# AbbVie-ComputationalGenomics/SAIGEgds

Measured on AMD Instinct MI355X. Metric: variants/sec seqAssocGLMM_SPA at N=430K; achieved HBM GB/s vs roofline, higher is better.
Workload: dtype f64

## Files before the change

### saigegds_amd/csrc/host_init.h

```cpp
extern "C" const char *sgx_version(void) { return "saigehip 0.1 (gfx950)"; }
extern "C" const char *sgx_last_error(void) { return g_err.c_str(); }

extern "C" int sgx_device_count(void)
{
	int n = 0;
	if (hipGetDeviceCount(&n) != hipSuccess) return 0;
	return n;
}

extern "C" size_t sgx_row_stride(int32_t n_samp)
{
	return (size_t)((n_samp + 511) / 512) * 128;
}

static double thr_or(double v, double dflt) { return std::isfinite(v) ? v : dflt; }

extern "C" int sgx_set_thresholds(sgx_handle *h, double maf, double mac, double missing,
	double spa_pval)
{
	if (!h) return fail(SGX_EINVAL, "sgx_set_thresholds: NULL handle");
	h->md.thr_maf = thr_or(maf, -1);
	h->md.thr_mac = thr_or(mac, -1);
	h->md.thr_missing = thr_or(missing, 1);
	h->md.thr_spa = thr_or(spa_pval, 0.05);
// ... 148 lines not shown
		return fail(SGX_EINVAL, "sgx_init: device %d out of range (0..%d)", device, ndev - 1);

	sgx_handle *h = new sgx_handle();
	h->device = device;
	int rc = set_dev(h);
	if (rc) { delete h; return rc; }
	const int P = 2 * K + 2;
	const bool quant = m->trait == SGX_TRAIT_QUANT;
	const int KP = (K + 2) & ~1;
	std::vector<double> F((size_t)N * P), X((size_t)N * K), y(m->y, m->y + N),
		mu(m->mu, m->mu + N), mu2(m->mu2, m->mu2 + N), XM((size_t)N * KP, 0.0);
	long double xmu[KMAX] = {0}, xsum[KMAX] = {0};
	for (int i = 0; i < N; i++) {
		const double w = quant ? 1.0 : m->mu2[i];
		double *f = &F[(size_t)i * P];
		for (int k = 0; k < K; k++) {
			f[k] = m->t_XVX_inv_XV[(size_t)i * K + k];
			f[K + k] = w * m->t_X[(size_t)i * K + k];
			X[(size_t)i * K + k] = m->t_X[(size_t)i * K + k];
			XM[(size_t)i * KP + k] = m->t_X[(size_t)i * K + k];
			xmu[k] += (long double)m->t_X[(size_t)i * K + k] * m->mu[i];
			xsum[k] += (long double)m->t_X[(size_t)i * K + k];
		}
		XM[(size_t)i * KP + K] = m->mu[i];
		f[2 * K] = m->y_mu[i];
		f[2 * K + 1] = w;
	}
	std::vector<int8_t> Fl;
	std::vector<long long> Qt;
	if ((double)N * 4.0 * 384.0 < 2147483647.0) {
		MfEpi &ep = h->mfe;
		const int CS = 2 * K, CW = 2 * K + 1;
		const int ngrp = (N + 15) / 16;
		const int ntile = 2 * ((ngrp + 31) / 32);
		const size_t ngrp_pad = (size_t)ntile * 16;
		ep.derive_c = quant && fit_xvx_inverse(m, ep.XVXi) ? 1 : 0;
		std::vector<int> order = {CS, CW};
		for (int k = 0; k < K; k++) order.push_back(K + k);
		if (!ep.derive_c) for (int k = 0; k < K; k++) order.push_back(k);
		for (int k = 0; k < K; k++) { ep.cgrp[k] = 0; ep.ccol[k] = 0; ep.climb[k] = 0; }
		bool range_ok = true;
		auto limbs_for = [&](int c) -> int {
			if (c == CW && quant) return 1;
			long double sum = 0; double mx = 0;
			for (int i = 0; i < N; i++) { const double a = std::fabs(F[(size_t)i * P + c]); sum += a; mx = std::max(mx, a); }
			const double range = sum > 0 ? mx / (double)(sum / N) : 1.0;
			if (!(range <= 4194304.0)) range_ok = false;
			int nl = c >= 2 * K ? MF_NLIMB : (c >= K ? MF_LIMB_E : MF_LIMB_A);
			if (range > 64.0) nl = std::max(nl, MF_LIMB_E);
			if (range > 16384.0) nl = MF_NLIMB;
			if (N < 16384) nl = std::min(MF_NLIMB, nl + 1);
			return nl;
		};
		int used = 1;
		for (int c : order) {
			const int nl = limbs_for(c);
			ep.cgrp[c] = 0; ep.ccol[c] = (unsigned char)(used - 1); ep.climb[c] = (unsigned char)nl;
			used += nl;
		}
		if (range_ok) {
		const int nbfv = (used + 15) / 16;
		h->mf_nbfv[0] = nbfv;
		ep.ngroups = 1;
		ep.goff[0] = 0;
		ep.gncol[0] = 16 * (nbfv + 1);
		ep.acc_stride = ep.gncol[0];
		ep.col_ones = used - 1;
		ep.col_b1 = 16 * nbfv;
		h->mf[0].ntile = ntile;
		Fl.assign(ngrp_pad * ep.gncol[0] * 16, 0);
		Qt.assign((size_t)N * P, 0);
		auto at = [&](int i, int col) -> int8_t & {
			return Fl[((size_t)(i / 16) * ep.gncol[0] + col) * 16 + s3_pos(i % 16)];
		};
		for (int c = 0; c < P; c++) {
			const int cc = ep.ccol[c], nl = ep.climb[c];
			if (nl == 0) { ep.escale[c] = 0; ep.ftot_hi[c] = ep.ftot_lo[c] = 0; continue; }
			double mx = 0;
			for (int i = 0; i < N; i++) mx = std::max(mx, std::fabs(F[(size_t)i * P + c]));
			int ex = 0;
			if (mx > 0) (void)std::frexp(mx, &ex);
			ep.escale[c] = (quant && c == CW) ? 2 : 8 * nl - 2 - ex;
			__int128 tot = 0;
			for (int i = 0; i < N; i++) {
				const int sc = s3_scale(i % 16);
				const long long d0 = std::llrint(std::ldexp(F[(size_t)i * P + c], ep.escale[c]) / sc);
				const long long q = d0 * sc;
				Qt[(size_t)i * P + c] = q;
				tot += q;
				long long rem = d0;
				for (int l = 0; l < nl; l++) {
					long long d = (l < nl - 1) ? (((rem + 128) & 255) - 128) : rem;
					rem = (rem - d) >> 8;
					at(i, cc + l) = (int8_t)d;
					if (c == CW) at(i, ep.col_b1 + l) = (int8_t)d;
				}
			}
			const __int128 two32 = ((__int128)1) << 32;
			__int128 hi = tot / two32, lo = tot - hi * two32;
			if (lo < 0) { lo += two32; hi -= 1; }
			ep.ftot_hi[c] = (long long)hi; ep.ftot_lo[c] = (long long)lo;
		}
		for (int i = 0; i < N; i++) {
			const int8_t d = (int8_t)(4 / s3_scale(i % 16));
			at(i, ep.col_ones) = d;
			at(i, ep.col_b1 + ep.climb[CW]) = d;
		}
		h->mf_ok = true;
		}
	}
	DevModel &md = h->md;
	md.N = N; md.K = K; md.P = P; md.quant = quant;
	md.tau0 = m->tau[0]; md.r = m->var_ratio;
	sgx_set_thresholds(h, m->maf, m->mac, m->missing, m->spa_pval);
	{
		double l2min = INFINITY;
		for (int i = 0; i < N; i++) {
			const double mi = m->mu[i];
			if (mi > 0 && mi < 1) { const double lg = std::log(mi / (1 - mi)); l2min = std::min(l2min, lg * lg); }
		}
		md.spa_xmax = std::isfinite(l2min) ? 0.25 * std::sqrt(l2min + M_PI * M_PI) : 0.0;
	}
	for (int k = 0; k < K; k++) {
		double mx = 0;
		for (int i = 0; i < N; i++) mx = std::max(mx, std::fabs(m->t_X[(size_t)i * K + k]));
		md.Xabs[k] = mx;
	}
	for (int a = 0; a < K * K; a++) md.XVX[a] = m->XVX[a];
	for (int a = 0; a < K; a++) { md.S_a[a] = m->S_a[a]; md.Xmu[a] = (double)xmu[a]; md.Xsum[a] = (double)xsum[a]; }
#define TRY(x) do { rc = (x); if (rc) { sgx_free(h); return rc; } } while (0)
	TRY(dev_upload(&h->dF, F));
	TRY(dev_upload(&h->dX, X));
	TRY(dev_upload(&h->dy, y));
	TRY(dev_upload(&h->dmu, mu));
	TRY(dev_upload(&h->dmu2, mu2));
	TRY(dev_upload(&h->dXM, XM));
	if (h->mf_ok) {
		std::vector<uint8_t> Flu(Fl.begin(), Fl.end());
		TRY(dev_upload(&h->dFl, Flu));
		h->mf[0].Fl = h->dFl;
		TRY(dev_upload(&h->dQ, Qt));
	}
	md.F = h->dF; md.X = h->dX; md.y = h->dy; md.mu = h->dmu; md.mu2 = h->dmu2; md.XM = h->dXM;
	rc = alloc_workspace(h);
	if (rc) { sgx_free(h); return rc; }
#undef TRY
	*out = h;
	return SGX_OK;
}

extern "C" int sgx_score_layout(sgx_handle *h, int32_t *limbs, int32_t n_limbs, int32_t *n_groups)
{
	if (!h || !n_groups) return fail(SGX_EINVAL, "sgx_score_layout: NULL argument");
	*n_groups = h->mf_ok ? h->mfe.ngroups : 0;
	for (int c = 0; limbs && c < n_limbs; c++) limbs[c] = (h->mf_ok && c < h->md.P) ? h->mfe.climb[c] : 0;
	return SGX_OK;
}

extern "C" void sgx_free(sgx_handle *h)
// ... 69 lines not shown
```

### saigegds_amd/csrc/kern_score3.h

```cpp
#pragma once
#include <type_traits>

#ifndef S3_V4I_DEFINED
#define S3_V4I_DEFINED
typedef int s3_v4i __attribute__((ext_vector_type(4)));
#endif

#include "s3_layout.h"

template <int OFF> __device__ __forceinline__ void s3_ds_read(s3_v4i &dst, uint32_t addr)
{
	asm volatile("ds_read_b128 %0, %1 offset:%2" : "=v"(dst) : "v"(addr), "n"(OFF));
}
template <int N> __device__ __forceinline__ void s3_lgkm_wait(s3_v4i &reg) { asm volatile("s_waitcnt lgkmcnt(%1)" : "+v"(reg) : "n"(N)); }
__device__ __forceinline__ void s3_tie(s3_v4i &reg) { asm volatile("" : "+v"(reg)); }
#define S3_DS_READ(dst, addr, off) s3_ds_read<(off)>(dst, addr)
#define S3_LGKM_WAIT(n, reg) s3_lgkm_wait<(n)>(reg)
#define S3_TIE(reg) s3_tie(reg)

template <int I, int N, typename F>
__device__ __forceinline__ void s3_static_for(F &&f)
{
	if constexpr (I < N) { f(std::integral_constant<int, I>()); s3_static_for<I + 1, N>(f); }
}

#ifndef S3_AUX_ROWS
#define S3_AUX_ROWS 2
#endif
#define S3_WAITCNT_VM(n) __builtin_amdgcn_s_waitcnt(((n) & 0xF) | (((n) >> 4) << 14) | (0x7 << 4) | (0xF << 8))

template <int OP>
__device__ __forceinline__ void s3_unpack_op(uint32_t w, uint32_t &w4, s3_v4i &val, s3_v4i &b1)
{
	if constexpr (OP == 0) w4 = w >> 4;
	else if constexpr (OP == 1) val[0] = (int)(w & 0x03030303u);
	else if constexpr (OP == 2) val[1] = (int)(w & 0x0C0C0C0Cu);
	else if constexpr (OP == 3) val[2] = (int)(w4 & 0x03030303u);
	else if constexpr (OP == 4) val[3] = (int)(w4 & 0x0C0C0C0Cu);
	else if constexpr (OP == 5) b1[0] = (int)(w & 0x02020202u);
	else if constexpr (OP == 6) b1[1] = (int)(w & 0x08080808u);
	else if constexpr (OP == 7) b1[2] = (int)(w4 & 0x02020202u);
	else if constexpr (OP == 8) b1[3] = (int)(w4 & 0x08080808u);
}
#define S3_UNPACK3_OPS 15
template <int OP>
__device__ __forceinline__ void s3_unpack3_op(uint32_t w, uint32_t &w4, uint32_t &t, uint32_t &t4, s3_v4i &val, s3_v4i &b1, s3_v4i &mis)
{
	if constexpr (OP < 9) s3_unpack_op<OP>(w, w4, val, b1);
	else if constexpr (OP == 9) t = w >> 1;
	else if constexpr (OP == 10) t4 = w4 >> 1;
	else if constexpr (OP == 11) mis[0] = (int)(w & t & 0x01010101u);
	else if constexpr (OP == 12) mis[1] = (int)(w & t & 0x04040404u);
	else if constexpr (OP == 13) mis[2] = (int)(w4 & t4 & 0x01010101u);
	else if constexpr (OP == 14) mis[3] = (int)(w4 & t4 & 0x04040404u);
}

template <int NAF>
struct s3_one {
	static constexpr int NM = 7 * NAF, NOPT = S3_UNPACK3_OPS * NAF, DL = 2, NK = 3 * NOPT;
	static constexpr int piece_of(int m) { return m < NAF ? m : m < 3 * NAF ? (m - NAF) / 2 : (m - 3 * NAF) / 4; }
	static constexpr int frag_of(int m) { return m < NAF ? 3 : m < 3 * NAF ? 0 : 1 + ((m - 3 * NAF) & 3) / 2; }
	static constexpr int plane_of(int m) { return m < NAF ? 2 : m < 3 * NAF ? (m - NAF) & 1 : (m - 3 * NAF) & 1; }
	static constexpr int chunk_of(int m) { return m < 3 * NAF ? 0 : 1; }
	static constexpr int slot_of(int m) { return m < NAF ? 0 : m < 3 * NAF ? 1 : ((m - 3 * NAF) & 3) / 2; }
	static constexpr int frag(int ch, int j) { return ch == 0 ? (j == 0 ? 3 : 0) : 1 + j; }
	static constexpr bool enters(int m) { return m == 0 || m == 3 * NAF; }
	static constexpr int piece(int i) { return i < 7 * NAF ? i / 7 : (i - 7 * NAF) / 8; }
	static constexpr int op(int i)
	{
		const int head[7] = {0, 9, 10, 5, 6, 7, 8}, tail[8] = {1, 2, 3, 4, 11, 12, 13, 14};
		return i < 7 * NAF ? head[i % 7] : tail[(i - 7 * NAF) % 8];
	}
	static constexpr int earliest(int d, int i)
	{
		const int base = NM * (d - 1);
		if (i < 7 * NAF) return base + (i % 7 >= 3 ? i / 7 : 0);
		const int q = i - 7 * NAF;
		return base + 3 * NAF + 4 * (q / 8) + (q % 8 < 4 ? 2 : 3);
	}
	static constexpr int deadline(int d, int i)
	{
		const int base = NM * d;
		if (i < 7 * NAF) return i % 7 >= 3 ? base + i / 7 : 1 << 30;
		const int q = i - 7 * NAF;
		return base + NAF + 2 * (q / 8) + (q % 8 < 4 ? 0 : 1);
	}
	static constexpr int slot(int k)
	{
		int s = 0;
		for (int j = 0; j <= k; j++) {
			const int d = 1 + j / NOPT, i = j % NOPT, t = NM * (d - 1) + i * NM / NOPT + DL, e = earliest(d, i);
			s = s > t ? s : t;
			s = s > e ? s : e;
		}
		return s;
	}
	static constexpr int first(int g) { int k = 0; while (k < NK && slot(k) < g) k++; return k; }
	static constexpr bool ok()
	{
		for (int k = 0; k < NK; k++)
			if (slot(k) >= deadline(1 + k / NOPT, k % NOPT) || slot(k) >= 4 * NM) return false;
		return true;
	}
};

template <int NBF, int NAF, int NC, int NLA, int NLB, int DA, int DB, int ABL = 0, int NCB = 1, int NBUF_ = 2, int RM = 0, bool MISS = false>
__global__ void __launch_bounds__(64 * (NC + NLA + NLB), (NC + NLA + NLB + 3) / 4)
score3_kernel(const uint8_t *__restrict__ A, const uint8_t *__restrict__ Fl, S3Plan pl, int *__restrict__ out, unsigned long long *__restrict__ stamps)
{
#if __HIP_DEVICE_COMPILE__
	static_assert(NC % NCB == 0 && NCB >= 1 && NCB <= 4, "consumer waves = variant groups x column groups");
	constexpr int NCV = NC / NCB;
	constexpr int NBWMAX = (NBF + NCB - 1) / NCB;
	constexpr int NCOL = 16 * NBF;
	constexpr int TILE_BYTES = 16 * NCOL * 16;
	constexpr int NPB = TILE_BYTES / 1024;
	constexpr int NPA = NCV * NAF;
	constexpr int RA = DA + 1, RB = DB + 1;
	constexpr int SLOT_A = (RM == 1 ? 2 : 1) * NPA * 1024;
	static_assert(DA >= 1 && DB >= 1, "at least one tile ahead");
	extern __shared__ __attribute__((aligned(16))) uint8_t s3_smem[];

	const int tid = threadIdx.x, lane = tid & 63, wid = tid >> 6;
	const int x = blockIdx.x & 7, y = blockIdx.x >> 3;
	const int g = x % pl.ng, i = y * (8 / pl.ng) + x / pl.ng;
	const int nk = pl.rf + (i < pl.rem * pl.f ? 1 : 0);
	const int T0 = 2 * (int)((long long)g * (pl.ntile / 2) / pl.ng), T1 = 2 * (int)((long long)(g + 1) * (pl.ntile / 2) / pl.ng);
	unsigned long long st0 = 0, sr0 = 0;
	if (ABL & 16) { st0 = __builtin_amdgcn_s_memtime(); sr0 = __builtin_amdgcn_s_memrealtime(); }

	struct Pos { int k, t, t1, vtile, id; };
	auto pos_set = [&](Pos &p, int k) {
		p.k = k;
		if (k >= nk) return;
		if (k < pl.rf) { p.vtile = k * pl.wpg + i; p.t = T0; p.t1 = T1; p.id = g * pl.ipg + p.vtile; }
		else {
			const int q = i % pl.f, vv = i / pl.f, len = T1 - T0;
			p.vtile = pl.rf * pl.wpg + vv;
			p.t = T0 + 2 * (q * (len / 2) / pl.f); p.t1 = T0 + 2 * ((q + 1) * (len / 2) / pl.f);
			p.id = g * pl.ipg + pl.rf * pl.wpg + i;
		}
	};
	auto pos_next = [&](Pos &p) { if (++p.t >= p.t1) pos_set(p, p.k + 1); };
	Pos pc;
	pos_set(pc, 0);

	if (wid >= NC) {
		const bool rows = wid < NC + NLA;
		const int l = __builtin_amdgcn_readfirstlane(rows ? wid - NC : wid - NC - NLA);
		const int voff = (rows ? s3_dma_lane(lane) : lane) * 16;
		const unsigned rm_bpv = (unsigned)pl.bpv;
		Pos pa = pc;
		int sl = 0;
		int ahead = 0;
		if (rows && RM == 1) {
			constexpr int PLO = NPA / NLA, NHI = NPA % NLA;
			static_assert(2 * (PLO + 1) * (DA > 1 ? DA - 1 : 1) < 64, "vmcnt range");
			const int li = lane >> 3, lj = lane & 7;
			const int rlast = pl.nrow - 1 - 16 * (pl.nfrag - 1);
			unsigned vo[2], vol[2];
#pragma unroll
			for (int h = 0; h < 2; h++) {
				const unsigned c = (unsigned)(lj ^ ((li >> 1) | (h << 2)));
				vo[h] = (unsigned)(8 * h + li) * rm_bpv + c * 16u;
				vol[h] = (unsigned)min(8 * h + li, rlast) * rm_bpv + c * 16u;
			}
			auto issue = [&]() {
// ... 54 lines not shown
#pragma unroll
			for (int d = 0; d < DA; d++) if (pa.k < nk) { issue(); ahead++; }
			while (pc.k < nk) {
				if (ahead == DA && DA > 1) { if (l < NHI) S3_WAITCNT_VM((PLO + 1) * (DA - 1)); else S3_WAITCNT_VM(PLO * (DA - 1)); }
				else S3_WAITCNT_VM(0);
				__builtin_amdgcn_s_barrier();
				ahead--;
				if (pa.k < nk) { issue(); ahead++; }
				pos_next(pc);
			}
		} else {
			constexpr int PLO = NPB / NLB, NHI = NPB % NLB;
			static_assert((PLO + 1) * (DB - 1) < 64, "vmcnt range");
			const __amdgpu_buffer_rsrc_t rsB = __builtin_amdgcn_make_buffer_rsrc((void *)Fl, 0, 0xFFFFFFFFu, 0x00020000);
			auto issue = [&]() {
#pragma unroll
				for (int j = 0; j <= PLO; j++) {
					const int b = l + j * NLB;
					if (b >= NPB || (ABL & 4)) break;
					__builtin_amdgcn_raw_ptr_buffer_load_lds(rsB, (__attribute__((address_space(3))) void *)(s3_smem + sl * TILE_BYTES + b * 1024),
						16, voff, pa.t * TILE_BYTES + b * 1024, 0, 0);
				}
				sl = sl + 1 == RB ? 0 : sl + 1;
				pos_next(pa);
			};
#pragma unroll
			for (int d = 0; d < DB; d++) if (pa.k < nk) { issue(); ahead++; }
			while (pc.k < nk) {
				if (ahead == DB && DB > 1) { if (l < NHI) S3_WAITCNT_VM((PLO + 1) * (DB - 1)); else S3_WAITCNT_VM(PLO * (DB - 1)); }
				else S3_WAITCNT_VM(0);
				__builtin_amdgcn_s_barrier();
				ahead--;
				if (pa.k < nk) { issue(); ahead++; }
				pos_next(pc);
			}
		}
		return;
	}

	const int r = lane & 15, kg = lane >> 4;
	const int vg = __builtin_amdgcn_readfirstlane(wid / NCB), cgr = __builtin_amdgcn_readfirstlane(wid % NCB);
	const uint32_t smem_lds = (uint32_t)(uintptr_t)(__attribute__((address_space(3))) uint8_t *)s3_smem;
	const uint32_t ring_lds = smem_lds + RB * TILE_BYTES + vg * (NAF * 1024) + lane * 16;
	const int rm_sig = ((r & 7) >> 1) | ((r >> 3) << 2);
	const uint32_t ring_rm = smem_lds + RB * TILE_BYTES + vg * (NAF * 2048) + (uint32_t)(r >> 3) * 1024u + (uint32_t)(r & 7) * 128u;
	const uint32_t ring_rm0 = ring_rm + (uint32_t)(kg ^ rm_sig) * 16u, ring_rm1 = ring_rm + (uint32_t)((4 + kg) ^ rm_sig) * 16u;

	auto consume = [&](auto CG) {
		constexpr int cg = decltype(CG)::value;
		constexpr int B0 = cg * NBWMAX;
		constexpr int NBW = (NBF - B0 < NBWMAX) ? NBF - B0 : NBWMAX;
		constexpr bool HASB1 = B0 + NBW == NBF;
		static_assert(NBW >= 1, "empty column group");
		const uint32_t bt_lds = smem_lds + (4 * kg * NCOL + r) * 16 + B0 * 256;

		s3_v4i acc[NAF][NBW];
#pragma unroll
		for (int f = 0; f < NAF; f++)
#pragma unroll
			for (int b = 0; b < NBW; b++) acc[f][b] = (s3_v4i){0, 0, 0, 0};

		constexpr int BCH = NBUF_ > 2 ? 1 : NCB > 1 ? (NBW <= 2 ? NBW : 2) : (NBF <= 4 ? NBF : (NBF >= 9 ? 2 : (NBF % 3 == 0 ? 3 : 4)));
		constexpr int NBUF = NBUF_;
		constexpr bool PIPE = NCB == 1 && NBF <= 8;
		constexpr int NCH = (NBW + BCH - 1) / BCH;
		constexpr int NM = NAF * NBW;
		constexpr int NV = HASB1 ? 4 * NAF : 0, NW = 5 * NAF;
		constexpr int BLV = HASB1 ? NBW - 2 : NBW - 1;
		constexpr int MB = HASB1 ? ((!PIPE && NBW >= 3) ? (NBW - 2) * NAF : (NBW - 1) * NAF) : 0;
		static_assert(!HASB1 || NBW >= 2 || NCB == 1, "a column group of the b1 fragment alone has no slot for its unpack");

		int sa = 0, sb = 0;
		int par = 0;
		while (pc.k < nk) {
			__builtin_amdgcn_sched_barrier(0);
			__builtin_amdgcn_s_barrier();
			__builtin_amdgcn_sched_barrier(0);
			const uint32_t a_addr = (RM == 1 ? (par ? ring_rm1 : ring_rm0) : ring_lds) + (uint32_t)(sa * SLOT_A);
			constexpr int AFS = RM == 1 ? 2048 : 1024;
			const uint32_t b_addr = bt_lds + (uint32_t)(sb * TILE_BYTES);
			s3_v4i aw[NAF];
			s3_static_for<0, NAF>([&](auto F) { constexpr int f = decltype(F)::value; S3_DS_READ(aw[f], a_addr, f * AFS); });
			s3_v4i bf[NBUF][BCH];
			auto read_chunk = [&](auto CI) {
				constexpr int ci = decltype(CI)::value, u = ci / NCH, b0 = (ci % NCH) * BCH;
				s3_static_for<0, BCH>([&](auto J) {
					constexpr int j = decltype(J)::value;
					if constexpr (b0 + j < NBW) {
						if (ABL & 8) bf[ci % NBUF][j] = (s3_v4i){u, j, r, sa};
						else S3_DS_READ(bf[ci % NBUF][j], b_addr, u * NCOL * 16 + (b0 + j) * 256);
					}
				});
			};
			constexpr int nread_last = NBW - (NCH - 1) * BCH;
			auto nreads = [](int c0, int c1) constexpr { int n = 0; for (int c = c0; c < c1 && c < 4 * NCH; c++) n += (c % NCH == NCH - 1) ? nread_last : BCH; return n; };
			s3_static_for<0, NBUF - 1>([&](auto C) { if constexpr (decltype(C)::value < 4 * NCH) read_chunk(C); });
			if (!(ABL & 8)) { S3_LGKM_WAIT(nreads(0, NBUF - 1), aw[0]); } else { S3_LGKM_WAIT(0, aw[0]); }
#pragma unroll
			for (int f = 1; f < NAF; f++) S3_TIE(aw[f]);
			s3_v4i val[PIPE ? 2 : 1][NAF], b1[NAF];
			uint32_t w4[PIPE ? 2 : 1][NAF];
			if (!(ABL & 1)) {
				s3_static_for<0, (PIPE ? NW : 5)>([&](auto O) {
					constexpr int o = decltype(O)::value, f = o / 5, op = o % 5;
					s3_unpack_op<op>((uint32_t)aw[f][0], w4[0][f], val[0][f], b1[f]);
				});
			}
			__builtin_amdgcn_sched_barrier(0);
			constexpr bool FM = !PIPE && BCH == 2 && nread_last == 2;
			constexpr int M0 = (NCH - 1) * BCH * NAF;
			s3_static_for<0, 4>([&](auto U) {
				constexpr int u = decltype(U)::value;
				constexpr int vb = PIPE ? (u & 1) : 0, vn = PIPE ? ((u + 1) & 1) : 0;
				s3_static_for<0, NM>([&](auto MI) {
					constexpr int m = decltype(MI)::value;
					constexpr bool fm = FM && m >= M0;
					constexpr int b = fm ? (NCH - 1) * BCH + (m - M0) % 2 : m / NAF, f = fm ? (m - M0) / 2 : m % NAF;
					constexpr int ch = b / BCH, ci = u * NCH + ch, j = b % BCH;
					if constexpr (m == ch * BCH * NAF) {
						if constexpr (ci + NBUF - 1 < 4 * NCH) read_chunk(std::integral_constant<int, ci + NBUF - 1>());
						constexpr int inflight = (ABL & 8) ? 0 : nreads(ci + 1, ci + NBUF);
						constexpr int nb = (ch == NCH - 1) ? nread_last : BCH;
						S3_LGKM_WAIT(inflight, bf[ci % NBUF][0]);
#pragma unroll
						for (int jj = 1; jj < nb; jj++) S3_TIE(bf[ci % NBUF][jj]);
					}
					if (ABL & 1) { if (f == 0) acc[0][b][1] ^= bf[ci % NBUF][j][0] ^ aw[b % NAF][u]; }
					else if (HASB1 && b == NBW - 1) acc[f][b] = __builtin_amdgcn_mfma_i32_16x16x64_i8(b1[f], bf[ci % NBUF][j], acc[f][b], 0, 0, 0);
					else acc[f][b] = __builtin_amdgcn_mfma_i32_16x16x64_i8(val[vb][f], bf[ci % NBUF][j], acc[f][b], 0, 0, 0);
					if (!(ABL & 1)) {
						if constexpr (!PIPE && u == 0 && b == 0 && f + 1 < NAF) {
							s3_static_for<0, 5>([&](auto O) {
								constexpr int op = decltype(O)::value;
								s3_unpack_op<op>((uint32_t)aw[f + 1][0], w4[0][f + 1], val[0][f + 1], b1[f + 1]);
							});
						}
						if constexpr (m < MB) {
							s3_static_for<m * NV / MB, (m + 1) * NV / MB>([&](auto O) {
								constexpr int o = decltype(O)::value, ff = o / 4, op = 5 + o % 4;
								s3_unpack_op<op>((uint32_t)aw[ff][u], w4[vb][ff], val[vb][ff], b1[ff]);
							});
						}
						if constexpr (PIPE && u < 3) {
							s3_static_for<m * NW / NM, (m + 1) * NW / NM>([&](auto O) {
								constexpr int o = decltype(O)::value, ff = o / 5, op = o % 5;
								s3_unpack_op<op>((uint32_t)aw[ff][u + 1], w4[vn][ff], val[vn][ff], b1[ff]);
							});
						}
						if constexpr (!PIPE && u < 3) {
							constexpr int lo = !fm ? ((b == BLV || (BLV < 0 && b == 0)) ? 0 : 5) : (HASB1 ? (j == 0 ? 0 : 2) : (j == 1 ? 0 : 5));
							constexpr int hi = !fm ? 5 : (HASB1 && j == 0 ? 2 : 5);
							s3_static_for<lo, hi>([&](auto O) {
								constexpr int op = decltype(O)::value;
								s3_unpack_op<op>((uint32_t)aw[f][u + 1], w4[0][f], val[0][f], b1[f]);
							});
						}
					}
					__builtin_amdgcn_sched_barrier(0);
				});
			});
			if (pc.t + 1 == pc.t1) {
				int *dst = out + ((size_t)pc.id * NC + wid) * (NAF * NBWMAX * 256) + lane;
#pragma unroll
				for (int f = 0; f < NAF; f++)
#pragma unroll
					for (int b = 0; b < NBW; b++)
#pragma unroll
						for (int reg = 0; reg < 4; reg++) {
							dst[((f * NBWMAX + b) * 4 + reg) * 64] = acc[f][b][reg];
							acc[f][b][reg] = 0;
						}
			}
			pos_next(pc);
			if (RM != 1 || par) sa = sa + 1 == RA ? 0 : sa + 1;
			sb = sb + 1 == RB ? 0 : sb + 1;
			par ^= 1;
		}
	};
	auto consume3 = [&]() {
		static_assert(!MISS || NCB == 1, "the three-plane form has one column group");
		constexpr int NBUF = NBUF_;
		constexpr int NBV = NBF - 1;
		constexpr int NVF = 2 * NBV + 1;
		constexpr int NM = NAF * NVF;
		constexpr int NOPT = S3_UNPACK3_OPS * NAF;
		constexpr bool ONE = NBF == 4 && NAF >= 3;
		using S1 = s3_one<NAF>;
		static_assert(!ONE || S1::ok(), "an unpack operation of the one-set schedule lands behind the MFMA that needs it");
		constexpr int BCH = ONE ? 2 : NBF <= 4 ? NBF : 2, NCH = (NBF + BCH - 1) / BCH;
		constexpr int NPS = ONE ? 1 : 2;
		const uint32_t bt_lds = smem_lds + (4 * kg * NCOL + r) * 16;
		s3_v4i acc[NAF][NBF], accm[NAF][NBV > 0 ? NBV : 1];
#pragma unroll
		for (int f = 0; f < NAF; f++) {
#pragma unroll
			for (int b = 0; b < NBF; b++) acc[f][b] = (s3_v4i){0, 0, 0, 0};
#pragma unroll
			for (int b = 0; b < NBV; b++) accm[f][b] = (s3_v4i){0, 0, 0, 0};
		}
		int sa = 0, sb = 0, par = 0;
		while (pc.k < nk) {
			__builtin_amdgcn_sched_barrier(0);
			__builtin_amdgcn_s_barrier();
			__builtin_amdgcn_sched_barrier(0);
			const uint32_t a_addr = (RM == 1 ? (par ? ring_rm1 : ring_rm0) : ring_lds) + (uint32_t)(sa * SLOT_A);
			constexpr int AFS = RM == 1 ? 2048 : 1024;
			const uint32_t b_addr = bt_lds + (uint32_t)(sb * TILE_BYTES);
			s3_v4i aw[NAF];
			s3_static_for<0, NAF>([&](auto F) { constexpr int f = decltype(F)::value; S3_DS_READ(aw[f], a_addr, f * AFS); });
			s3_v4i bf[NBUF][BCH];
			auto read_chunk = [&](auto CI) {
				constexpr int ci = decltype(CI)::value, u = ci / NCH, b0 = (ci % NCH) * BCH;
				s3_static_for<0, BCH>([&](auto J) {
					constexpr int j = decltype(J)::value;
					constexpr int b = ONE ? S1::frag(ci % NCH, j) : b0 + j;
					if constexpr (b0 + j < NBF) S3_DS_READ(bf[ci % NBUF][j], b_addr, u * NCOL * 16 + b * 256);
				});
			};
			constexpr int nread_last = NBF - (NCH - 1) * BCH;
			auto nreads = [](int c0, int c1) constexpr { int n = 0; for (int c = c0; c < c1 && c < 4 * NCH; c++) n += (c % NCH == NCH - 1) ? nread_last : BCH; return n; };
			s3_static_for<0, NBUF - 1>([&](auto C) { if constexpr (decltype(C)::value < 4 * NCH) read_chunk(C); });
			S3_LGKM_WAIT(nreads(0, NBUF - 1), aw[0]);
#pragma unroll
			for (int f = 1; f < NAF; f++) S3_TIE(aw[f]);
			s3_v4i val[NPS][NAF], b1[NPS][NAF], mis[NPS][NAF];
			uint32_t w4[NAF], tt[NAF], m4[NAF];
			s3_static_for<0, NOPT>([&](auto O) {
				constexpr int o = decltype(O)::value, f = o / S3_UNPACK3_OPS, op = o % S3_UNPACK3_OPS;
				s3_unpack3_op<op>((uint32_t)aw[f][0], w4[f], tt[f], m4[f], val[0][f], b1[0][f], mis[0][f]);
			});
			__builtin_amdgcn_sched_barrier(0);
			s3_static_for<0, 4>([&](auto U) {
				constexpr int u = decltype(U)::value, vb = ONE ? 0 : u & 1, vn = ONE ? 0 : (u + 1) & 1;
				s3_static_for<0, NM>([&](auto MI) {
					constexpr int m = decltype(MI)::value, vf = m / NAF;
					constexpr int f = ONE ? S1::piece_of(m) : m % NAF;
					constexpr int b = ONE ? S1::frag_of(m) : vf < 2 * NBV ? vf / 2 : NBV;
					constexpr int plane = ONE ? S1::plane_of(m) : vf < 2 * NBV ? (vf & 1) : 2;
					constexpr int ch = ONE ? S1::chunk_of(m) : b / BCH, ci = u * NCH + ch, j = ONE ? S1::slot_of(m) : b % BCH;
					if constexpr (ONE ? S1::enters(m) : f == 0 && plane != 1 && b % BCH == 0) {
						if constexpr (ci + NBUF - 1 < 4 * NCH) read_chunk(std::integral_constant<int, ci + NBUF - 1>());
						constexpr int inflight = nreads(ci + 1, ci + NBUF);
						constexpr int nb = (ch == NCH - 1) ? nread_last : BCH;
						S3_LGKM_WAIT(inflight, bf[ci % NBUF][0]);
#pragma unroll
						for (int jj = 1; jj < nb; jj++) S3_TIE(bf[ci % NBUF][jj]);
					}
					if constexpr (plane == 0) acc[f][b] = __builtin_amdgcn_mfma_i32_16x16x64_i8(val[vb][f], bf[ci % NBUF][j], acc[f][b], 0, 0, 0);
					else if constexpr (plane == 1) accm[f][b] = __builtin_amdgcn_mfma_i32_16x16x64_i8(mis[vb][f], bf[ci % NBUF][j], accm[f][b], 0, 0, 0);
					else acc[f][b] = __builtin_amdgcn_mfma_i32_16x16x64_i8(b1[vb][f], bf[ci % NBUF][j], acc[f][b], 0, 0, 0);
					if constexpr (ONE) {
						constexpr int g = u * NM + m;
						s3_static_for<S1::first(g), S1::first(g + 1)>([&](auto K) {
							constexpr int k = decltype(K)::value, d = 1 + k / NOPT, i = k % NOPT, ff = S1::piece(i), op = S1::op(i);
							s3_unpack3_op<op>((uint32_t)aw[ff][d], w4[ff], tt[ff], m4[ff], val[0][ff], b1[0][ff], mis[0][ff]);
						});
					} else if constexpr (u < 3) {
						s3_static_for<m * NOPT / NM, (m + 1) * NOPT / NM>([&](auto O) {
							constexpr int o = decltype(O)::value, ff = o / S3_UNPACK3_OPS, op = o % S3_UNPACK3_OPS;
							s3_unpack3_op<op>((uint32_t)aw[ff][u + 1], w4[ff], tt[ff], m4[ff], val[vn][ff], b1[vn][ff], mis[vn][ff]);
						});
					}
					__builtin_amdgcn_sched_barrier(0);
				});
			});
			if (pc.t + 1 == pc.t1) {
				int *dst = out + ((size_t)pc.id * NC + wid) * (NAF * NVF * 256) + lane;
#pragma unroll
				for (int f = 0; f < NAF; f++) {
#pragma unroll
					for (int b = 0; b < NBF; b++)
#pragma unroll
						for (int reg = 0; reg < 4; reg++) { dst[((f * NVF + b) * 4 + reg) * 64] = acc[f][b][reg]; acc[f][b][reg] = 0; }
#pragma unroll
					for (int b = 0; b < NBV; b++)
#pragma unroll
						for (int reg = 0; reg < 4; reg++) { dst[((f * NVF + NBF + b) * 4 + reg) * 64] = accm[f][b][reg]; accm[f][b][reg] = 0; }
				}
			}
			pos_next(pc);
			if (RM != 1 || par) sa = sa + 1 == RA ? 0 : sa + 1;
			sb = sb + 1 == RB ? 0 : sb + 1;
			par ^= 1;
		}
	};
	if constexpr (MISS) consume3();
	else if constexpr (NCB == 1) consume(std::integral_constant<int, 0>());
	else s3_static_for<0, NCB>([&](auto CG) { if (cgr == decltype(CG)::value) consume(CG); });
	if ((ABL & 16) && tid == 0) {
		stamps[2 * blockIdx.x] = __builtin_amdgcn_s_memtime() - st0;
		stamps[2 * blockIdx.x + 1] = __builtin_amdgcn_s_memrealtime() - sr0;
	}
#endif
}

#define S3_FOR_EACH_NBF(X) \
	X(2, 4, 8, 3, 1, 1, 2) X(3, 4, 8, 3, 1, 1, 1) X(4, 4, 8, 3, 1, 1, 1) X(5, 3, 8, 3, 1, 1, 2) X(6, 3, 8, 3, 1, 1, 1) \
	X(7, 4, 4, 2, 2, 2, 1) X(8, 4, 4, 2, 2, 2, 1) X(9, 4, 4, 2, 2, 1, 1) X(10, 4, 4, 2, 2, 1, 1) X(11, 4, 4, 2, 2, 1, 1) \
	X(12, 3, 4, 2, 2, 1, 1) X(13, 3, 4, 2, 2, 1, 1) X(14, 2, 4, 2, 2, 2, 1) X(15, 2, 4, 2, 2, 1, 1) X(16, 2, 4, 2, 2, 1, 1)
#define S3_FOR_EACH_NBF_MISS(X) \
	X(2, 4, 8, 3, 1, 1, 2) X(3, 3, 8, 3, 1, 1, 2) X(4, 3, 8, 3, 1, 1, 2) X(5, 2, 8, 3, 1, 2, 2) X(6, 3, 4, 2, 2, 2, 1) \
	X(7, 2, 4, 2, 2, 2, 1) X(8, 2, 4, 2, 2, 2, 1) X(9, 2, 4, 2, 2, 2, 1) X(10, 2, 4, 2, 2, 2, 1) X(11, 1, 4, 2, 2, 2, 1) \
	X(12, 1, 4, 2, 2, 2, 1) X(13, 1, 4, 2, 2, 2, 1) X(14, 1, 4, 2, 2, 2, 1) X(15, 1, 4, 2, 2, 2, 1) X(16, 1, 4, 2, 2, 2, 1)
static inline size_t s3_lds_bytes(int NBF, int NAF, int NC, int DA, int DB) { return ((size_t)(DB + 1) * 4 * NBF + (size_t)(DA + 1) * 2 * NC * NAF) * 1024; }

#ifndef S3_KERNEL_ONLY
#include "kern_lists.h"

__device__ __forceinline__ unsigned long long s3_block_excl(unsigned long long x, unsigned long long *sh)
{
	const int tid = threadIdx.x;
	sh[tid] = x;
	__syncthreads();
	for (int o = 1; o < 1024; o <<= 1) {
		const unsigned long long y = tid >= o ? sh[tid - o] : 0;
		__syncthreads();
		sh[tid] += y;
		__syncthreads();
	}
	const unsigned long long incl = sh[tid];
	__syncthreads();
	return incl - x;
}

__global__ void __launch_bounds__(256)
s3_ingest_clist_count_kernel(int M, int N, int lim, int *__restrict__ nzv ,
	const int *__restrict__ n2v, const int *__restrict__ n3, uint8_t *__restrict__ corient)
{
	const int v = blockIdx.x * 256 + threadIdx.x;
	if (v >= M) return;
	const int nz = nzv[v], n2 = n2v[v], m3 = n3[v];
	const long long AC = (long long)(nz - n2 - m3) + 2ll * n2;
	const bool minus = (double)AC / (2.0 * (double)(N - m3)) > 0.5;
	const int nnz = minus ? N - n2 : nz;
	const int orient = (N - m3 > 0 && nnz <= lim) ? (minus ? 2 : 1) : 0;
	corient[v] = (uint8_t)orient;
	nzv[v] = orient ? nnz : 0;
}

__global__ void __launch_bounds__(1024)
s3_ingest_clist_kernel(int M, unsigned cidx_cap, const int *__restrict__ cn, unsigned *__restrict__ cptr, uint8_t *__restrict__ corient)
{
	__shared__ unsigned long long sh[1024];
	const int tid = threadIdx.x, per = (M + 1023) / 1024, v0 = tid * per, v1 = min(M, v0 + per);
	unsigned long long mine = 0;
	for (int v = v0; v < v1; v++) mine += (unsigned long long)cn[v];
	unsigned long long base = s3_block_excl(mine, sh);
	for (int v = v0; v < v1; v++) {
		const int n = cn[v];
		const bool fits = base + (unsigned long long)n <= (unsigned long long)cidx_cap;
		cptr[v] = (unsigned)min(base, (unsigned long long)cidx_cap);
		if (!fits) corient[v] = 0;
		else base += (unsigned long long)n;
	}
	if (tid == 1023) cptr[M] = (unsigned)min(base, (unsigned long long)cidx_cap);
}

// ... 72 lines not shown
	const long long *__restrict__ t3part , int nr,
	const int *__restrict__ lcnt , size_t ld, int *__restrict__ ovf_list,
	SpaRec *__restrict__ recs, int *__restrict__ counters, int btop, int *__restrict__ fb_series, int *__restrict__ fb_exact,
	double *__restrict__ out8, uint8_t *__restrict__ valid, double guard_tol, int dbg = 0)
{
	constexpr int P = 2 * K + 2, CW = P - 1;
	constexpr int S3E_VB = s3e_vb(K);
	__shared__ double s_acc[S3E_VB][P | 1];
	__shared__ double s_imp[S3E_VB];
	__shared__ int s_n[S3E_VB][4];
	__shared__ long long s_ftot[P][2];
	__shared__ int s_col[P][3];
	const int tid = threadIdx.x, j0 = blockIdx.x * S3E_VB;
	const int N = md.N;
	if (dbg & 1) {
		if (tid == 0)
#pragma unroll
			for (int c = 0; c < P; c++) {
				s_col[c][0] = ep.ccol[c]; s_col[c][1] = ep.climb[c]; s_col[c][2] = ep.escale[c];
				s_ftot[c][0] = ep.ftot_hi[c]; s_ftot[c][1] = ep.ftot_lo[c];
			}
	} else
	for (int c = tid; c < P; c += S3E_VB) {
		s_col[c][0] = ep.ccol[c]; s_col[c][1] = ep.climb[c]; s_col[c][2] = ep.escale[c];
		s_ftot[c][0] = ep.ftot_hi[c]; s_ftot[c][1] = ep.ftot_lo[c];
	}
	{
		const int j = j0 + tid;
		const int *a0 = accbuf + (size_t)min(j, M - 1) * acc_stride;
		int n3 = 0;
		bool over = false;
		if (miss_off) n3 = a0[miss_off + ep.col_ones] / 4;
		else {
			for (int g0 = 0; g0 < nr; g0 += 8) {
				int cn[8];
#pragma unroll
				for (int u = 0; u < 8; u++) cn[u] = lcnt[(size_t)min(g0 + u, nr - 1) * ld + min(j, M - 1)];
#pragma unroll
				for (int u = 0; u < 8; u++) if (g0 + u < nr) { over |= cn[u] < 0; n3 += cn[u] < 0 ? 0 : cn[u]; }
			}
		}
		if (j >= M) n3 = 0;
		{
			const int tot = wave_total_i(n3);
			if ((tid & 63) == 0 && tot >= 64) atomicAdd(&counters[22], tot >> 6);
		}
		int state = 0, n1 = 0, n2 = 0;
		double imp = 0;
		if (dbg & 8) over = false;
		if (j < M) {
			if (over) ovf_list[atomicAdd(&counters[23], 1)] = j;
			else {
				const long long AC = (long long)(a0[ep.col_ones] / 4) - 3ll * n3;
				n2 = a0[ep.col_b1 + ep.climb[CW]] / 8 - n3;
				n1 = (int)(AC - 2ll * n2);
				const VarHead h = make_head(md, (double)AC, N - n3);
				if (!h.pass) { nan_row(out8 + (size_t)j * 8); valid[j] = 0; }
				else { state = h.minus ? 2 : 1; imp = 2 * h.AF; }
			}
		}
		s_n[tid][0] = n1; s_n[tid][1] = n2; s_n[tid][2] = n3; s_n[tid][3] = state;
		s_imp[tid] = imp;
	}
	__syncthreads();
	for (int task = tid; task < S3E_VB * P; task += S3E_VB) {
		const int vl = task / P, c = task - vl * P, j = j0 + vl;
		const int state = s_n[vl][3];
		if (!state) continue;
		const int cc = s_col[c][0], nl = s_col[c][1];
		if (nl == 0) { s_acc[vl][c] = 0; continue; }
		const int *a0 = accbuf + (size_t)j * acc_stride;
		const bool minus = state == 2;
		const double imp = s_imp[vl];
		int lv[MF_NLIMB], lm[MF_NLIMB], lb[MF_NLIMB];
#pragma unroll
		for (int l = 0; l < MF_NLIMB; l++) lv[l] = a0[cc + min(l, nl - 1)];
		HiLo T3 = hl(0, 0);
		if (miss_off) {
#pragma unroll
			for (int l = 0; l < MF_NLIMB; l++) lm[l] = a0[miss_off + cc + min(l, nl - 1)];
		} else if (!(dbg & 2)) {
			const long long *p = t3part + ((size_t)j * P + c) * 2;
			const size_t gs = (size_t)M * P * 2;
			for (int g0 = 0; g0 < nr; g0 += 8) {
				long long ph[8], pl[8];
#pragma unroll
				for (int u = 0; u < 8; u++) { const long long *q = p + (size_t)min(g0 + u, nr - 1) * gs; ph[u] = q[0]; pl[u] = q[1]; }
#pragma unroll
				for (int u = 0; u < 8; u++) if (g0 + u < nr) { T3.hi += ph[u]; T3.lo += pl[u]; }
			}
		}
		if (c == CW) {
#pragma unroll
			for (int l = 0; l < MF_NLIMB; l++) lb[l] = a0[ep.col_b1 + min(l, nl - 1)];
		}
		auto limbs = [&](const int (&x)[MF_NLIMB]) -> HiLo {
			long long lo = 0, hi = 0;
#pragma unroll
			for (int l = 3; l >= 0; l--) lo = lo * 256 + (l < nl ? x[l] : 0);
#pragma unroll
			for (int l = MF_NLIMB - 1; l >= 4; l--) hi = hi * 256 + (l < nl ? x[l] : 0);
			return hl(hi, lo);
		};
		const HiLo V = limbs(lv);
		if (miss_off) T3 = limbs(lm);
		const HiLo W = hl_axpy(-3, T3, V);
		const double t3d = hl_to_double(T3);
// ... 93 lines not shown
```

### saigegds_amd/csrc/kern_score_mfma.h

```cpp
#pragma once
#include <type_traits>


typedef int v4i __attribute__((ext_vector_type(4)));

#define MF_NAF 4
#ifndef MF_WAVES
#define MF_WAVES 4
#endif
#define MF_VPW (16 * MF_NAF)
#define MF_VPB (MF_VPW * MF_WAVES)
#define MF_NLIMB 7
#define MF_LIMB_A 5
#define MF_LIMB_E 6
#define MF_GLIMBS 64
#define MF_MAXP (2 * SGX_MAX_COEFF + 2)
#define MF_MAXG 4

struct MfTab {
	const uint8_t *Fl;
	int ntile;
};

struct MfEpi {
	int ngroups, acc_stride;
	int goff[MF_MAXG], gncol[MF_MAXG];
	int col_ones;
	int col_b1;
	unsigned char cgrp[MF_MAXP], ccol[MF_MAXP], climb[MF_MAXP];
	int derive_c;
	double XVXi[SGX_MAX_COEFF * SGX_MAX_COEFF];
	int escale[MF_MAXP];
	long long ftot_hi[MF_MAXP];
	long long ftot_lo[MF_MAXP];
};

__host__ __device__ __forceinline__ int mf_pos(int s) { return ((s & 3) << 2) | (s >> 2); }

__device__ __forceinline__ void mf_unpack(uint32_t w, v4i &val, v4i &b1)
{
	val[0] = (int)(w & 0x03030303u);
	val[1] = (int)((w >> 2) & 0x03030303u);
	val[2] = (int)((w >> 4) & 0x03030303u);
	val[3] = (int)((w >> 6) & 0x03030303u);
#pragma unroll
	for (int k = 0; k < 4; k++) b1[k] = (int)((uint32_t)val[k] & 0x02020202u);
}

template <int NBFV, bool HAS_B1, bool WIDE = false, int ABL = 0, int NAF = MF_NAF>
__global__ void __launch_bounds__(WAVE * MF_WAVES, NAF == 4 ? 2 : NAF == 3 ? 3 : 4)
score_mfma_kernel(const uint8_t *__restrict__ packed, size_t bpv, int M, MfTab tb,
	int tiles_per_split, int *__restrict__ accbuf, int acc_stride)
{
	constexpr int NBF = NBFV + (HAS_B1 ? 1 : 0);
	constexpr int NCOL = 16 * NBF;
	constexpr int TILE_BYTES = 16 * NCOL * 16;
	constexpr int NDMA = (TILE_BYTES / 1024 + MF_WAVES - 1) / MF_WAVES;
	constexpr int AW = WIDE ? 2 : 1;
	constexpr bool SPREAD = !(ABL & (2048 | 16));
	static_assert(AW * NAF + NDMA <= 4 * NAF, "more loads per tile than MFMA groups");
	extern __shared__ __attribute__((aligned(16))) uint8_t smem[];
	uint8_t *ldsB = smem;

	const int tid = threadIdx.x, lane = tid & (WAVE - 1), wid = tid / WAVE;
	const int r = lane & 15, kg = lane >> 4;
	unsigned vt_idx = blockIdx.x, split = blockIdx.y;
	{
		const unsigned VT = gridDim.x, L = blockIdx.y * VT + blockIdx.x, full = gridDim.y & ~7u;
		if (L < full * VT) { const unsigned q = L >> 3; split = 8 * (q / VT) + (L & 7); vt_idx = q % VT; }
	}
	const int vbase = vt_idx * (16 * NAF * MF_WAVES) + wid * 16 * NAF;
	const int t0 = split * tiles_per_split;
	const int t1 = min(tb.ntile, t0 + tiles_per_split);

	v4i acc[NAF][NBF], accm[NAF][NBFV];
#pragma unroll
	for (int f = 0; f < NAF; f++) {
#pragma unroll
		for (int b = 0; b < NBF; b++) acc[f][b] = (v4i){0, 0, 0, 0};
#pragma unroll
		for (int b = 0; b < NBFV; b++) accm[f][b] = (v4i){0, 0, 0, 0};
// ... 170 lines not shown
```

Before: 18.42 million.

## Drop duplicated bit-1 fragment from B tile by reusing value fragment 0

The host layout no longer stores a separate bit-1 copy of the weight and constant columns. The constant column is placed right after the weight limbs so both sit in value fragment 0. The kernels now read fragment 0 again for the bit-1 MFMAs, with optional register aliasing, instead of loading a dedicated fragment. This cuts B-tile bytes, LDS footprint and ds_reads per tile, at the cost of a more involved compile-time schedule and a new init failure when the constant column falls outside fragment 0.

```diff
diff --git a/saigegds_amd/csrc/host_init.h b/saigegds_amd/csrc/host_init.h
--- a/saigegds_amd/csrc/host_init.h
+++ b/saigegds_amd/csrc/host_init.h
@@ -224,12 +224,14 @@
 			if (N < 16384) nl = std::min(MF_NLIMB, nl + 1);
 			return nl;
 		};
-		int used = 1;
+		int used = 0, col_ones = -1;
 		for (int c : order) {
 			const int nl = limbs_for(c);
-			ep.cgrp[c] = 0; ep.ccol[c] = (unsigned char)(used - 1); ep.climb[c] = (unsigned char)nl;
+			ep.cgrp[c] = 0; ep.ccol[c] = (unsigned char)used; ep.climb[c] = (unsigned char)nl;
 			used += nl;
-		}
+			if (c == CW) col_ones = used++;
+		}
+		if (col_ones < 0 || col_ones >= 16) { delete h; return fail(SGX_EINVAL, "sgx_init: the constant column (%d) is outside value fragment 0", col_ones); }
 		if (range_ok) {
 		const int nbfv = (used + 15) / 16;
 		h->mf_nbfv[0] = nbfv;
@@ -237,13 +239,15 @@
 		ep.goff[0] = 0;
 		ep.gncol[0] = 16 * (nbfv + 1);
 		ep.acc_stride = ep.gncol[0];
-		ep.col_ones = used - 1;
-		ep.col_b1 = 16 * nbfv;
+		ep.col_ones = col_ones;
+		ep.col_b1 = 16 * nbfv + ep.ccol[CW];
+		ep.col_b1_ones = 16 * nbfv + col_ones;
 		h->mf[0].ntile = ntile;
-		Fl.assign(ngrp_pad * ep.gncol[0] * 16, 0);
+		const size_t ncolB = 16 * (size_t)nbfv;
+		Fl.assign(ngrp_pad * ncolB * 16, 0);
 		Qt.assign((size_t)N * P, 0);
 		auto at = [&](int i, int col) -> int8_t & {
-			return Fl[((size_t)(i / 16) * ep.gncol[0] + col) * 16 + s3_pos(i % 16)];
+			return Fl[((size_t)(i / 16) * ncolB + col) * 16 + s3_pos(i % 16)];
 		};
 		for (int c = 0; c < P; c++) {
 			const int cc = ep.ccol[c], nl = ep.climb[c];
@@ -265,7 +269,6 @@
 					long long d = (l < nl - 1) ? (((rem + 128) & 255) - 128) : rem;
 					rem = (rem - d) >> 8;
 					at(i, cc + l) = (int8_t)d;
-					if (c == CW) at(i, ep.col_b1 + l) = (int8_t)d;
 				}
 			}
 			const __int128 two32 = ((__int128)1) << 32;
@@ -276,7 +279,6 @@
 		for (int i = 0; i < N; i++) {
 			const int8_t d = (int8_t)(4 / s3_scale(i % 16));
 			at(i, ep.col_ones) = d;
-			at(i, ep.col_b1 + ep.climb[CW]) = d;
 		}
 		h->mf_ok = true;
 		}
diff --git a/saigegds_amd/csrc/kern_score3.h b/saigegds_amd/csrc/kern_score3.h
--- a/saigegds_amd/csrc/kern_score3.h
+++ b/saigegds_amd/csrc/kern_score3.h
@@ -59,11 +59,11 @@
 struct s3_one {
 	static constexpr int NM = 7 * NAF, NOPT = S3_UNPACK3_OPS * NAF, DL = 2, NK = 3 * NOPT;
 	static constexpr int piece_of(int m) { return m < NAF ? m : m < 3 * NAF ? (m - NAF) / 2 : (m - 3 * NAF) / 4; }
-	static constexpr int frag_of(int m) { return m < NAF ? 3 : m < 3 * NAF ? 0 : 1 + ((m - 3 * NAF) & 3) / 2; }
+	static constexpr int frag_of(int m) { return m < 3 * NAF ? 0 : 1 + ((m - 3 * NAF) & 3) / 2; }
 	static constexpr int plane_of(int m) { return m < NAF ? 2 : m < 3 * NAF ? (m - NAF) & 1 : (m - 3 * NAF) & 1; }
 	static constexpr int chunk_of(int m) { return m < 3 * NAF ? 0 : 1; }
-	static constexpr int slot_of(int m) { return m < NAF ? 0 : m < 3 * NAF ? 1 : ((m - 3 * NAF) & 3) / 2; }
-	static constexpr int frag(int ch, int j) { return ch == 0 ? (j == 0 ? 3 : 0) : 1 + j; }
+	static constexpr int slot_of(int m) { return m < 3 * NAF ? 0 : ((m - 3 * NAF) & 3) / 2; }
+	static constexpr int frag(int ch, int j) { return ch == 0 ? 0 : 1 + j; }
 	static constexpr bool enters(int m) { return m == 0 || m == 3 * NAF; }
 	static constexpr int piece(int i) { return i < 7 * NAF ? i / 7 : (i - 7 * NAF) / 8; }
 	static constexpr int op(int i)
@@ -104,6 +104,9 @@
 	}
 };
 
+constexpr int s3_slot_at(bool early, int nbw, int p) { return !early ? p : p == 0 ? 0 : p == 1 ? nbw - 1 : p - 1; }
+constexpr int s3_chunk_n(bool one, int nch, int bch, int nlast, int ch) { return one ? (ch == 0 ? 1 : 2) : ch == nch - 1 ? nlast : bch; }
+
 template <int NBF, int NAF, int NC, int NLA, int NLB, int DA, int DB, int ABL = 0, int NCB = 1, int NBUF_ = 2, int RM = 0, bool MISS = false>
 __global__ void __launch_bounds__(64 * (NC + NLA + NLB), (NC + NLA + NLB + 3) / 4)
 score3_kernel(const uint8_t *__restrict__ A, const uint8_t *__restrict__ Fl, S3Plan pl, int *__restrict__ out, unsigned long long *__restrict__ stamps)
@@ -111,8 +114,10 @@
 #if __HIP_DEVICE_COMPILE__
 	static_assert(NC % NCB == 0 && NCB >= 1 && NCB <= 4, "consumer waves = variant groups x column groups");
 	constexpr int NCV = NC / NCB;
+	static_assert(NBF >= 2, "a value fragment and the bit-1 slot");
+	constexpr int NBV = NBF - 1;
 	constexpr int NBWMAX = (NBF + NCB - 1) / NCB;
-	constexpr int NCOL = 16 * NBF;
+	constexpr int NCOL = 16 * NBV;
 	constexpr int TILE_BYTES = 16 * NCOL * 16;
 	constexpr int NPB = TILE_BYTES / 1024;
 	constexpr int NPA = NCV * NAF;
@@ -273,7 +278,7 @@
 		constexpr int NBW = (NBF - B0 < NBWMAX) ? NBF - B0 : NBWMAX;
 		constexpr bool HASB1 = B0 + NBW == NBF;
 		static_assert(NBW >= 1, "empty column group");
-		const uint32_t bt_lds = smem_lds + (4 * kg * NCOL + r) * 16 + B0 * 256;
+		const uint32_t bt_lds = smem_lds + (4 * kg * NCOL + r) * 16;
 
 		s3_v4i acc[NAF][NBW];
 #pragma unroll
@@ -286,9 +291,14 @@
 		constexpr bool PIPE = NCB == 1 && NBF <= 8;
 		constexpr int NCH = (NBW + BCH - 1) / BCH;
 		constexpr int NM = NAF * NBW;
+		constexpr bool SHARE = HASB1 && B0 == 0;
+		constexpr bool EARLY = SHARE && NCH > 1;
+		constexpr int PB1 = !HASB1 ? -1 : EARLY ? 1 : NBW - 1;
+		constexpr bool ALIAS = SHARE && PB1 < BCH;
+		constexpr bool LASTB1 = HASB1 && !EARLY;
 		constexpr int NV = HASB1 ? 4 * NAF : 0, NW = 5 * NAF;
-		constexpr int BLV = HASB1 ? NBW - 2 : NBW - 1;
-		constexpr int MB = HASB1 ? ((!PIPE && NBW >= 3) ? (NBW - 2) * NAF : (NBW - 1) * NAF) : 0;
+		constexpr int BLV = LASTB1 ? NBW - 2 : NBW - 1;
+		constexpr int MB = EARLY ? NAF : HASB1 ? ((!PIPE && NBW >= 3) ? (NBW - 2) * NAF : (NBW - 1) * NAF) : 0;
 		static_assert(!HASB1 || NBW >= 2 || NCB == 1, "a column group of the b1 fragment alone has no slot for its unpack");
 
 		int sa = 0, sb = 0;
@@ -307,14 +317,19 @@
 				constexpr int ci = decltype(CI)::value, u = ci / NCH, b0 = (ci % NCH) * BCH;
 				s3_static_for<0, BCH>([&](auto J) {
 					constexpr int j = decltype(J)::value;
-					if constexpr (b0 + j < NBW) {
+					if constexpr (b0 + j < NBW && !(ALIAS && b0 + j == PB1)) {
+						constexpr int frag = b0 + j == PB1 ? 0 : B0 + s3_slot_at(EARLY, NBW, b0 + j);
 						if (ABL & 8) bf[ci % NBUF][j] = (s3_v4i){u, j, r, sa};
-						else S3_DS_READ(bf[ci % NBUF][j], b_addr, u * NCOL * 16 + (b0 + j) * 256);
+						else S3_DS_READ(bf[ci % NBUF][j], b_addr, u * NCOL * 16 + frag * 256);
 					}
 				});
 			};
 			constexpr int nread_last = NBW - (NCH - 1) * BCH;
-			auto nreads = [](int c0, int c1) constexpr { int n = 0; for (int c = c0; c < c1 && c < 4 * NCH; c++) n += (c % NCH == NCH - 1) ? nread_last : BCH; return n; };
+			auto nreads = [](int c0, int c1) constexpr {
+				int n = 0;
+				for (int c = c0; c < c1 && c < 4 * NCH; c++) n += ((c % NCH == NCH - 1) ? nread_last : BCH) - ((ALIAS && c % NCH == 0) ? 1 : 0);
+				return n;
+			};
 			s3_static_for<0, NBUF - 1>([&](auto C) { if constexpr (decltype(C)::value < 4 * NCH) read_chunk(C); });
 			if (!(ABL & 8)) { S3_LGKM_WAIT(nreads(0, NBUF - 1), aw[0]); } else { S3_LGKM_WAIT(0, aw[0]); }
 #pragma unroll
@@ -336,21 +351,22 @@
 				s3_static_for<0, NM>([&](auto MI) {
 					constexpr int m = decltype(MI)::value;
 					constexpr bool fm = FM && m >= M0;
-					constexpr int b = fm ? (NCH - 1) * BCH + (m - M0) % 2 : m / NAF, f = fm ? (m - M0) / 2 : m % NAF;
-					constexpr int ch = b / BCH, ci = u * NCH + ch, j = b % BCH;
+					constexpr int p = fm ? (NCH - 1) * BCH + (m - M0) % 2 : m / NAF, f = fm ? (m - M0) / 2 : m % NAF;
+					constexpr int b = s3_slot_at(EARLY, NBW, p);
+					constexpr int ch = p / BCH, ci = u * NCH + ch, j = (ALIAS && p == PB1) ? 0 : p % BCH;
 					if constexpr (m == ch * BCH * NAF) {
 						if constexpr (ci + NBUF - 1 < 4 * NCH) read_chunk(std::integral_constant<int, ci + NBUF - 1>());
 						constexpr int inflight = (ABL & 8) ? 0 : nreads(ci + 1, ci + NBUF);
 						constexpr int nb = (ch == NCH - 1) ? nread_last : BCH;
 						S3_LGKM_WAIT(inflight, bf[ci % NBUF][0]);
 #pragma unroll
-						for (int jj = 1; jj < nb; jj++) S3_TIE(bf[ci % NBUF][jj]);
+						for (int jj = 1; jj < nb; jj++) if (!(ALIAS && ch == 0 && jj == PB1)) S3_TIE(bf[ci % NBUF][jj]);
 					}
 					if (ABL & 1) { if (f == 0) acc[0][b][1] ^= bf[ci % NBUF][j][0] ^ aw[b % NAF][u]; }
-					else if (HASB1 && b == NBW - 1) acc[f][b] = __builtin_amdgcn_mfma_i32_16x16x64_i8(b1[f], bf[ci % NBUF][j], acc[f][b], 0, 0, 0);
+					else if (p == PB1) acc[f][b] = __builtin_amdgcn_mfma_i32_16x16x64_i8(b1[f], bf[ci % NBUF][j], acc[f][b], 0, 0, 0);
 					else acc[f][b] = __builtin_amdgcn_mfma_i32_16x16x64_i8(val[vb][f], bf[ci % NBUF][j], acc[f][b], 0, 0, 0);
 					if (!(ABL & 1)) {
-						if constexpr (!PIPE && u == 0 && b == 0 && f + 1 < NAF) {
+						if constexpr (!PIPE && u == 0 && p == 0 && f + 1 < NAF) {
 							s3_static_for<0, 5>([&](auto O) {
 								constexpr int op = decltype(O)::value;
 								s3_unpack_op<op>((uint32_t)aw[f + 1][0], w4[0][f + 1], val[0][f + 1], b1[f + 1]);
@@ -369,8 +385,8 @@
 							});
 						}
 						if constexpr (!PIPE && u < 3) {
-							constexpr int lo = !fm ? ((b == BLV || (BLV < 0 && b == 0)) ? 0 : 5) : (HASB1 ? (j == 0 ? 0 : 2) : (j == 1 ? 0 : 5));
-							constexpr int hi = !fm ? 5 : (HASB1 && j == 0 ? 2 : 5);
+							constexpr int lo = !fm ? ((p == BLV || (BLV < 0 && p == 0)) ? 0 : 5) : (LASTB1 ? (j == 0 ? 0 : 2) : (j == 1 ? 0 : 5));
+							constexpr int hi = !fm ? 5 : (LASTB1 && j == 0 ? 2 : 5);
 							s3_static_for<lo, hi>([&](auto O) {
 								constexpr int op = decltype(O)::value;
 								s3_unpack_op<op>((uint32_t)aw[f][u + 1], w4[0][f], val[0][f], b1[f]);
@@ -401,14 +417,14 @@
 	auto consume3 = [&]() {
 		static_assert(!MISS || NCB == 1, "the three-plane form has one column group");
 		constexpr int NBUF = NBUF_;
-		constexpr int NBV = NBF - 1;
 		constexpr int NVF = 2 * NBV + 1;
 		constexpr int NM = NAF * NVF;
 		constexpr int NOPT = S3_UNPACK3_OPS * NAF;
 		constexpr bool ONE = NBF == 4 && NAF >= 3;
 		using S1 = s3_one<NAF>;
 		static_assert(!ONE || S1::ok(), "an unpack operation of the one-set schedule lands behind the MFMA that needs it");
-		constexpr int BCH = ONE ? 2 : NBF <= 4 ? NBF : 2, NCH = (NBF + BCH - 1) / BCH;
+		constexpr int BCH = ONE ? 2 : NBV <= 3 ? NBV : 2, NCH = ONE ? 2 : (NBV + BCH - 1) / BCH;
+		constexpr int NLAST = NBV - (NCH - 1) * BCH;
 		constexpr int NPS = ONE ? 1 : 2;
 		const uint32_t bt_lds = smem_lds + (4 * kg * NCOL + r) * 16;
 		s3_v4i acc[NAF][NBF], accm[NAF][NBV > 0 ? NBV : 1];
@@ -432,14 +448,13 @@
 			s3_v4i bf[NBUF][BCH];
 			auto read_chunk = [&](auto CI) {
 				constexpr int ci = decltype(CI)::value, u = ci / NCH, b0 = (ci % NCH) * BCH;
-				s3_static_for<0, BCH>([&](auto J) {
+				s3_static_for<0, s3_chunk_n(ONE, NCH, BCH, NLAST, ci % NCH)>([&](auto J) {
 					constexpr int j = decltype(J)::value;
 					constexpr int b = ONE ? S1::frag(ci % NCH, j) : b0 + j;
-					if constexpr (b0 + j < NBF) S3_DS_READ(bf[ci % NBUF][j], b_addr, u * NCOL * 16 + b * 256);
+					S3_DS_READ(bf[ci % NBUF][j], b_addr, u * NCOL * 16 + b * 256);
 				});
 			};
-			constexpr int nread_last = NBF - (NCH - 1) * BCH;
-			auto nreads = [](int c0, int c1) constexpr { int n = 0; for (int c = c0; c < c1 && c < 4 * NCH; c++) n += (c % NCH == NCH - 1) ? nread_last : BCH; return n; };
+			auto nreads = [](int c0, int c1) constexpr { int n = 0; for (int c = c0; c < c1 && c < 4 * NCH; c++) n += s3_chunk_n(ONE, NCH, BCH, NLAST, c % NCH); return n; };
 			s3_static_for<0, NBUF - 1>([&](auto C) { if constexpr (decltype(C)::value < 4 * NCH) read_chunk(C); });
 			S3_LGKM_WAIT(nreads(0, NBUF - 1), aw[0]);
 #pragma unroll
@@ -456,20 +471,20 @@
 				s3_static_for<0, NM>([&](auto MI) {
 					constexpr int m = decltype(MI)::value, vf = m / NAF;
 					constexpr int f = ONE ? S1::piece_of(m) : m % NAF;
-					constexpr int b = ONE ? S1::frag_of(m) : vf < 2 * NBV ? vf / 2 : NBV;
-					constexpr int plane = ONE ? S1::plane_of(m) : vf < 2 * NBV ? (vf & 1) : 2;
+					constexpr int b = ONE ? S1::frag_of(m) : vf < 3 ? 0 : 1 + (vf - 3) / 2;
+					constexpr int plane = ONE ? S1::plane_of(m) : vf < 3 ? vf : (vf - 3) & 1;
 					constexpr int ch = ONE ? S1::chunk_of(m) : b / BCH, ci = u * NCH + ch, j = ONE ? S1::slot_of(m) : b % BCH;
-					if constexpr (ONE ? S1::enters(m) : f == 0 && plane != 1 && b % BCH == 0) {
+					if constexpr (ONE ? S1::enters(m) : f == 0 && plane == 0 && b % BCH == 0) {
 						if constexpr (ci + NBUF - 1 < 4 * NCH) read_chunk(std::integral_constant<int, ci + NBUF - 1>());
 						constexpr int inflight = nreads(ci + 1, ci + NBUF);
-						constexpr int nb = (ch == NCH - 1) ? nread_last : BCH;
+						constexpr int nb = s3_chunk_n(ONE, NCH, BCH, NLAST, ch);
 						S3_LGKM_WAIT(inflight, bf[ci % NBUF][0]);
 #pragma unroll
 						for (int jj = 1; jj < nb; jj++) S3_TIE(bf[ci % NBUF][jj]);
 					}
 					if constexpr (plane == 0) acc[f][b] = __builtin_amdgcn_mfma_i32_16x16x64_i8(val[vb][f], bf[ci % NBUF][j], acc[f][b], 0, 0, 0);
 					else if constexpr (plane == 1) accm[f][b] = __builtin_amdgcn_mfma_i32_16x16x64_i8(mis[vb][f], bf[ci % NBUF][j], accm[f][b], 0, 0, 0);
-					else acc[f][b] = __builtin_amdgcn_mfma_i32_16x16x64_i8(b1[vb][f], bf[ci % NBUF][j], acc[f][b], 0, 0, 0);
+					else acc[f][NBV] = __builtin_amdgcn_mfma_i32_16x16x64_i8(b1[vb][f], bf[ci % NBUF][j], acc[f][NBV], 0, 0, 0);
 					if constexpr (ONE) {
 						constexpr int g = u * NM + m;
 						s3_static_for<S1::first(g), S1::first(g + 1)>([&](auto K) {
@@ -523,7 +538,7 @@
 	X(2, 4, 8, 3, 1, 1, 2) X(3, 3, 8, 3, 1, 1, 2) X(4, 3, 8, 3, 1, 1, 2) X(5, 2, 8, 3, 1, 2, 2) X(6, 3, 4, 2, 2, 2, 1) \
 	X(7, 2, 4, 2, 2, 2, 1) X(8, 2, 4, 2, 2, 2, 1) X(9, 2, 4, 2, 2, 2, 1) X(10, 2, 4, 2, 2, 2, 1) X(11, 1, 4, 2, 2, 2, 1) \
 	X(12, 1, 4, 2, 2, 2, 1) X(13, 1, 4, 2, 2, 2, 1) X(14, 1, 4, 2, 2, 2, 1) X(15, 1, 4, 2, 2, 2, 1) X(16, 1, 4, 2, 2, 2, 1)
-static inline size_t s3_lds_bytes(int NBF, int NAF, int NC, int DA, int DB) { return ((size_t)(DB + 1) * 4 * NBF + (size_t)(DA + 1) * 2 * NC * NAF) * 1024; }
+static inline size_t s3_lds_bytes(int NBF, int NAF, int NC, int DA, int DB) { return ((size_t)(DB + 1) * 4 * (NBF - 1) + (size_t)(DA + 1) * 2 * NC * NAF) * 1024; }
 
 #ifndef S3_KERNEL_ONLY
 #include "kern_lists.h"
@@ -702,7 +717,7 @@
 			if (over) ovf_list[atomicAdd(&counters[23], 1)] = j;
 			else {
 				const long long AC = (long long)(a0[ep.col_ones] / 4) - 3ll * n3;
-				n2 = a0[ep.col_b1 + ep.climb[CW]] / 8 - n3;
+				n2 = a0[ep.col_b1_ones] / 8 - n3;
 				n1 = (int)(AC - 2ll * n2);
 				const VarHead h = make_head(md, (double)AC, N - n3);
 				if (!h.pass) { nan_row(out8 + (size_t)j * 8); valid[j] = 0; }
diff --git a/saigegds_amd/csrc/kern_score_mfma.h b/saigegds_amd/csrc/kern_score_mfma.h
--- a/saigegds_amd/csrc/kern_score_mfma.h
+++ b/saigegds_amd/csrc/kern_score_mfma.h
@@ -27,6 +27,7 @@
 	int goff[MF_MAXG], gncol[MF_MAXG];
 	int col_ones;
 	int col_b1;
+	int col_b1_ones;
 	unsigned char cgrp[MF_MAXP], ccol[MF_MAXP], climb[MF_MAXP];
 	int derive_c;
 	double XVXi[SGX_MAX_COEFF * SGX_MAX_COEFF];
```

New measurement: 17.88 million. 2.9% lower.
